# psipred/DMPfold2

Measured on AMD Instinct MI355X. Metric: structures/s at L=300, N_seq=2000, 10 iters+100 min, higher is better.
Workload: dtype f32 with full-width operands on the bf16 matrix cores (option precision = 2): convolution operands split exactly into 3 bf16 pieces (24 significand bits), the 6 piece products above 2^-24 accumulated in f32 by v_mfma_f32_32x32x16_bf16; vertical GRU the same way (3 bf16 pieces per operand, 6 products

## Files before the change

dmpfold2_amd/csrc/vgru_x3.hip:

```cpp
#include "vgru.h"

namespace dmp {

typedef __bf16 vx_bf16x8 __attribute__((ext_vector_type(8)));

__device__ __forceinline__ void vx_split8(const float (&w)[8], vx_bf16x8 (&p)[3]) {
  float r[8];
#pragma unroll
  for (int e = 0; e < 8; ++e) { const __bf16 h = (__bf16)w[e]; p[0][e] = h; r[e] = w[e] - (float)h; }
#pragma unroll
  for (int e = 0; e < 8; ++e) { const __bf16 h = (__bf16)r[e]; p[1][e] = h; r[e] = r[e] - (float)h; }
#pragma unroll
  for (int e = 0; e < 8; ++e) p[2][e] = (__bf16)r[e];
}

__device__ __forceinline__ vp_f32x4 vx_mfma(vx_bf16x8 a, vx_bf16x8 b, vp_f32x4 c) {
  return __builtin_amdgcn_mfma_f32_16x16x32_bf16(a, b, c, 0, 0, 0);
}

__device__ __forceinline__ float vx_sigmoid(float x) { return 1.0f / (1.0f + expf(-x)); }

constexpr int VX_KS = 4;
constexpr int VX_WQ = 6;
constexpr size_t VX_WQ_BYTES = (size_t)VP_GRID * 4 * VX_KS * VX_WQ * 64 * 16;
static_assert(4 * VX_KS * 3 * 2 * 64 == VP_WL0_SLOTS, "two pieces of layer 0's weights fill the LDS area of the f16 form's pieces");

constexpr int VX_SC1 = 16;

struct VxAddr {
  __amdgpu_buffer_rsrc_t r0, r1, rq;
  unsigned vlane, vq;
  unsigned k4w, krot, Lb;
};

__device__ __forceinline__ void vx_request(vp_f32x4 (&F)[4][2], int u4, unsigned S, unsigned col, const VxAddr& A) {
  const unsigned base = ((A.k4w + 8 * ((S + A.krot) & (VX_KS - 1))) * A.Lb + col + (u4 & 1) * 16) * 16;
#pragma unroll
  for (int h = 0; h < 2; ++h)
    F[u4][h] = __builtin_bit_cast(vp_f32x4, __builtin_amdgcn_raw_buffer_load_b128(u4 < 2 ? A.r1 : A.r0, A.vlane, base + h * A.Lb * 16, VX_SC1));
}

__device__ __forceinline__ void vx_split_octet(const vp_f32x4 (&f)[2], vx_bf16x8 (&q)[3]) {
  const float wv[8] = {f[0][0], f[0][1], f[0][2], f[0][3], f[1][0], f[1][1], f[1][2], f[1][3]};
  vx_split8(wv, q);
}

template <bool ACT0, bool ACT1>
__device__ __forceinline__ void vx_tile_products(vp_f32x4 (&a0)[3][2], vp_f32x4 (&a1)[4][2], const vx_bf16x8 (&PA)[VX_KS][3][3],
                                                 const vx_bf16x8 (&PB)[VX_KS][3][2], vx_bf16x8 (&WB)[3], vx_bf16x8 (&WC)[3],
                                                 const vx_bf16x8* __restrict__ wl0w, vp_f32x4 (&F)[4][2], vx_bf16x8 (&Q)[2][3],
                                                 const VxAddr& A, unsigned tcol, unsigned ncol) {
#pragma unroll
  for (int S = 0; S < VX_KS; ++S) {
    vx_bf16x8 T[3][2];
#pragma unroll
    for (int g = 0; g < 3; ++g) {
      T[g][0] = wl0w[((S * 3 + g) * 2 + 0) * 64];
      T[g][1] = wl0w[((S * 3 + g) * 2 + 1) * 64];
    }
    __builtin_amdgcn_sched_barrier(0);
#pragma unroll
    for (int u4 = 0; u4 < 4; ++u4) {
      const int unit = 4 * S + u4, nt = u4 & 1, cur = unit & 1, nxt = cur ^ 1, n4 = (u4 + 1) & 3;
      vx_bf16x8 (&P)[3] = Q[cur];
      const int nm = u4 < 2 ? (ACT1 ? 18 : 0) : (ACT0 ? 18 : 0) + (ACT1 ? 18 : 0);
#pragma unroll
      for (int pb = 2; pb >= 0; --pb)
#pragma unroll
        for (int pa = 2 - pb; pa >= 0; --pa)
#pragma unroll
          for (int g = 0; g < 3; ++g) {
            if (u4 < 2) {
              if (ACT1) a1[g][nt] = vx_mfma(pa == 2 ? WB[g] : PB[S][g][pa == 2 ? 0 : pa], P[pb], a1[g][nt]);
            } else {
              if (ACT0) a0[g][nt] = vx_mfma(pa == 2 ? WC[g] : T[g][pa == 2 ? 0 : pa], P[pb], a0[g][nt]);
              if (ACT1) a1[g == 2 ? 3 : g][nt] = vx_mfma(PA[S][g][pa], P[pb], a1[g == 2 ? 3 : g][nt]);
            }
          }
      vx_split_octet(F[n4], Q[nxt]);
      vx_request(F, n4, (unit + 5) >> 2 & (VX_KS - 1), unit + 5 < 4 * VX_KS ? tcol : ncol, A);
      if (u4 == 1) {
#pragma unroll
        for (int g = 0; g < 3; ++g)
          WB[g] = __builtin_bit_cast(vx_bf16x8, __builtin_amdgcn_raw_buffer_load_b128(A.rq, A.vq, (((S + 1) & (VX_KS - 1)) * VX_WQ + g) * 1024, 0));
      }
      if (u4 == 3) {
#pragma unroll
        for (int g = 0; g < 3; ++g)
          WC[g] = __builtin_bit_cast(vx_bf16x8, __builtin_amdgcn_raw_buffer_load_b128(A.rq, A.vq, (((S + 1) & (VX_KS - 1)) * VX_WQ + 3 + g) * 1024, 0));
      }
#pragma unroll
      for (int i = 0; i < 36; ++i)
        if (i < nm) {
          __builtin_amdgcn_sched_group_barrier(0x008, 1, 0);
          __builtin_amdgcn_sched_group_barrier(0x002, 3, 0);
        }
      __builtin_amdgcn_sched_barrier(0);
    }
  }
}

__global__ __launch_bounds__(256) __attribute__((amdgpu_waves_per_eu(1, 1)))
void vgru_persist_x3_kernel(VStaticF32 st, const VGroupRec* __restrict__ rec, VPSync* __restrict__ sync,
                            int* __restrict__ fault, int t_lo, int t_hi, int ntiles, int barrier) {
  extern __shared__ __attribute__((aligned(16))) unsigned char vx_smem[];
  vx_bf16x8* wl0 = reinterpret_cast<vx_bf16x8*>(vx_smem);
  vp_f32x4* red = reinterpret_cast<vp_f32x4*>(vx_smem + VP_WL0_SLOTS * 16);
  float* tab = reinterpret_cast<float*>(vx_smem + (VP_WL0_SLOTS + VP_RED_SLOTS) * 16);
  __shared__ int sh_u, sh_abort;
  __shared__ __attribute__((aligned(16))) float sh_bias[2][4][16];
  __shared__ int sh_tile[VP_MAX_XCD_TILES][5];
  __shared__ unsigned long long sh_msa[VG_MAX_MEMBERS];
  const int tid = threadIdx.x, lane = tid & 63;
  const int w = __builtin_amdgcn_readfirstlane(tid >> 6);
  unsigned xcc;
  if (barrier) {
    asm volatile("s_getreg_b32 %0, hwreg(HW_REG_XCC_ID)" : "=s"(xcc));
    xcc &= 7u;
    if (tid == 0) {
      sh_u = (int)__hip_atomic_fetch_add(&sync->count[xcc], 1u, __ATOMIC_RELAXED, __HIP_MEMORY_SCOPE_AGENT);
      sh_abort = 0;
    }
  } else {
    xcc = blockIdx.x & 7u;
    if (tid == 0) { sh_u = (int)(blockIdx.x >> 3); sh_abort = 0; }
  }
  __syncthreads();
  const int u = sh_u;
  if (u >= 32) {
    if (tid == 0) atomicOr(fault, DMP_FAULT_VGRU_HANDOFF);
    return;
  }
  const int j0 = 16 * u, lr = lane & 15, lq = lane >> 4;
  const int Lb = ntiles * VG_TB;
  const int c_lo = (int)(((long long)ntiles * xcc) / 8), c_hi = (int)(((long long)ntiles * (xcc + 1)) / 8);

  vx_bf16x8 PA[VX_KS][3][3], PB[VX_KS][3][2];
  uint4* wqw = st.wq + (size_t)(blockIdx.x * 4 + w) * VX_KS * VX_WQ * 64 + lane;
#pragma unroll
  for (int S = 0; S < VX_KS; ++S)
#pragma unroll
    for (int g = 0; g < 3; ++g) {
      float wa[8], wb[8], wc[8];
#pragma unroll
      for (int h = 0; h < 2; ++h) {
        const int64_t off = (int64_t)(g * 128 + 32 * w + 8 * ((S + u) & (VX_KS - 1)) + 2 * lq + h) * 512 + j0 + lr;
        const float4 a = st.wx1[off], b = st.wh1[off], c = st.wh0[off];
        wa[4 * h + 0] = a.x; wa[4 * h + 1] = a.y; wa[4 * h + 2] = a.z; wa[4 * h + 3] = a.w;
        wb[4 * h + 0] = b.x; wb[4 * h + 1] = b.y; wb[4 * h + 2] = b.z; wb[4 * h + 3] = b.w;
        wc[4 * h + 0] = c.x; wc[4 * h + 1] = c.y; wc[4 * h + 2] = c.z; wc[4 * h + 3] = c.w;
      }
      vx_split8(wa, PA[S][g]);
      vx_bf16x8 pb[3], pc[3];
      vx_split8(wb, pb);
      vx_split8(wc, pc);
      PB[S][g][0] = pb[0];
      PB[S][g][1] = pb[1];
      wl0[(((w * VX_KS + S) * 3 + g) * 2 + 0) * 64 + lane] = pc[0];
      wl0[(((w * VX_KS + S) * 3 + g) * 2 + 1) * 64 + lane] = pc[1];
      wqw[(S * VX_WQ + g) * 64] = __builtin_bit_cast(uint4, pb[2]);
      wqw[(S * VX_WQ + 3 + g) * 64] = __builtin_bit_cast(uint4, pc[2]);
    }
  asm volatile("s_waitcnt vmcnt(0)" ::: "memory");
  const vx_bf16x8* wl0w = wl0 + w * VX_KS * 3 * 2 * 64 + lane;
  if (tid < 128) sh_bias[tid >> 6][(tid >> 4) & 3][tid & 15] = st.bias[tid >> 6][((tid >> 4) & 3) * 512 + j0 + (tid & 15)];
  for (int i = tid; i < 3 * 22 * 16; i += 256) {
    const int g = i / (22 * 16), code = (i / 16) % 22, row = i & 15;
    tab[(g * 24 + code) * 16 + row] = st.wx0[(g * 22 + code) * 512 + j0 + row];
  }
  const int fl = __builtin_amdgcn_readfirstlane(tid >> 7), fg = (tid >> 5) & 3, fc = tid & 31;
  const int flane = 16 * fg + (fc & 15), fnt = fc >> 4;
  const int j4 = j0 + 4 * fg;
  const int nmem = rec->nmem;
  if (c_hi - c_lo > VP_MAX_XCD_TILES) {
    if (tid == 0) atomicOr(fault, DMP_FAULT_VGRU_HANDOFF);
    return;
  }
  for (int i = tid; i < c_hi - c_lo; i += 256) {
    const int tile = c_lo + (i + u) % (c_hi - c_lo);
    int mi = 0;
    for (int m = 1; m < VG_MAX_MEMBERS; ++m)
      if (m < nmem && tile >= rec->mem[m].tile0) mi = m;
    sh_tile[i][0] = rec->mem[mi].N;
    sh_tile[i][1] = rec->mem[mi].L;
    sh_tile[i][2] = (tile - rec->mem[mi].tile0) * VG_TB;
    sh_tile[i][3] = mi;
    sh_tile[i][4] = tile;
  }
  if (tid < VG_MAX_MEMBERS) sh_msa[tid] = tid < nmem ? (unsigned long long)rec->mem[tid].msa : 0ull;
  __syncthreads();
  auto next_active = [&](int ct, int t) {
    for (; ct < c_hi; ++ct) {
      const int N = __builtin_amdgcn_readfirstlane(sh_tile[ct - c_lo][0]);
      if (t < N || (t >= 1 && t <= N)) break;
    }
    return ct;
  };
  const unsigned state_bytes = (unsigned)(128 * Lb * 16);

  VxAddr A;
  A.k4w = (unsigned)(32 * w);
  A.krot = (unsigned)(u & (VX_KS - 1));
  A.Lb = (unsigned)Lb;
  A.vlane = (unsigned)((2 * lq * Lb + lr) * 16);
  A.vq = (unsigned)(lane * 16);
  A.rq = __builtin_amdgcn_make_buffer_rsrc(st.wq + (size_t)(blockIdx.x * 4 + w) * VX_KS * VX_WQ * 64, 0, VX_KS * VX_WQ * 1024, 0x00020000);
  vx_bf16x8 WB[3], WC[3];
#pragma unroll
  for (int g = 0; g < 3; ++g) {
    WB[g] = __builtin_bit_cast(vx_bf16x8, __builtin_amdgcn_raw_buffer_load_b128(A.rq, A.vq, g * 1024, 0));
    WC[g] = __builtin_bit_cast(vx_bf16x8, __builtin_amdgcn_raw_buffer_load_b128(A.rq, A.vq, (3 + g) * 1024, 0));
  }
  for (int t = t_lo; t < t_hi; ++t) {
    const int par = t & 1;
    A.r0 = __builtin_amdgcn_make_buffer_rsrc(st.hT[0][par], 0, state_bytes, 0x00020000);
    A.r1 = __builtin_amdgcn_make_buffer_rsrc(st.hT[1][par ^ 1], 0, state_bytes, 0x00020000);
    const __amdgpu_buffer_rsrc_t rh = fl ? A.r1 : A.r0;
    float* hnext = fl ? st.hT[1][par] : st.hT[0][par ^ 1];
    int ct = next_active(c_lo, t);
    vp_f32x4 F[4][2];
    vx_bf16x8 Q[2][3];
    if (ct < c_hi) {
      const unsigned col0 = (unsigned)(__builtin_amdgcn_readfirstlane(sh_tile[ct - c_lo][4]) * VG_TB);
#pragma unroll
      for (int u4 = 0; u4 < 4; ++u4) vx_request(F, u4, 0, col0, A);
      vx_split_octet(F[0], Q[0]);
      vx_request(F, 0, 1, col0, A);
    }
    while (ct < c_hi) {
      const int nx = next_active(ct + 1, t);
      const int ncol = __builtin_amdgcn_readfirstlane(sh_tile[(nx < c_hi ? nx : ct) - c_lo][4]) * VG_TB;
      const int N = __builtin_amdgcn_readfirstlane(sh_tile[ct - c_lo][0]);
      const int L = __builtin_amdgcn_readfirstlane(sh_tile[ct - c_lo][1]);
      const bool act0 = t < N, act1 = t >= 1 && t <= N;
      const int tcol = __builtin_amdgcn_readfirstlane(sh_tile[ct - c_lo][4]) * VG_TB;
      vp_f32x4 a0[3][2], a1[4][2];
#pragma unroll
      for (int g = 0; g < 3; ++g) { a0[g][0] = vp_f32x4{0, 0, 0, 0}; a0[g][1] = vp_f32x4{0, 0, 0, 0}; }
#pragma unroll
      for (int g = 0; g < 4; ++g) { a1[g][0] = vp_f32x4{0, 0, 0, 0}; a1[g][1] = vp_f32x4{0, 0, 0, 0}; }
      if (act0 && act1)
        vx_tile_products<true, true>(a0, a1, PA, PB, WB, WC, wl0w, F, Q, A, (unsigned)tcol, (unsigned)ncol);
      else if (act0)
        vx_tile_products<true, false>(a0, a1, PA, PB, WB, WC, wl0w, F, Q, A, (unsigned)tcol, (unsigned)ncol);
      else
        vx_tile_products<false, true>(a0, a1, PA, PB, WB, WC, wl0w, F, Q, A, (unsigned)tcol, (unsigned)ncol);
      const int b = tcol + fc;
      const int64_t hoff = ((int64_t)(j4 >> 2) * Lb + b) * 4;
      float hp[4];
#pragma unroll
      for (int i = 0; i < 4; ++i)
        hp[i] = __builtin_bit_cast(float, __builtin_amdgcn_raw_buffer_load_b32(rh, (unsigned)(hoff * 4 + 4 * i), 0, VX_SC1));
      const int bm = sh_tile[ct - c_lo][2] + fc;
      const uint8_t* msa = reinterpret_cast<const uint8_t*>(sh_msa[sh_tile[ct - c_lo][3]]);
      const int code = (fl == 0 && act0 && bm < L) ? (int)msa[(int64_t)t * L + bm] : 0;
#pragma unroll
      for (int g = 0; g < 3; ++g)
#pragma unroll
        for (int nt = 0; nt < 2; ++nt) red[(w * 14 + g * 2 + nt) * 64 + lane] = a0[g][nt];
#pragma unroll
      for (int g = 0; g < 4; ++g)
#pragma unroll
        for (int nt = 0; nt < 2; ++nt) red[(w * 14 + 6 + g * 2 + nt) * 64 + lane] = a1[g][nt];
      __syncthreads();
      if (fl ? act1 : act0) {
        const int nq = fl ? 4 : 3, base = fl ? 6 : 0;
        vp_f32x4 sum[4];
#pragma unroll
        for (int q = 0; q < 4; ++q) {
          if (q < nq) {
            const int a = base + q * 2 + fnt;
            sum[q] = ((red[(0 * 14 + a) * 64 + flane] + red[(1 * 14 + a) * 64 + flane]) + red[(2 * 14 + a) * 64 + flane]) +
                     red[(3 * 14 + a) * 64 + flane];
          }
        }
        if (fl == 0) {
          const float* tr = tab + (0 * 24 + code) * 16 + 4 * fg;
          const float* tz = tab + (1 * 24 + code) * 16 + 4 * fg;
          const float* tn = tab + (2 * 24 + code) * 16 + 4 * fg;
#pragma unroll
          for (int i = 0; i < 4; ++i) { sum[0][i] += tr[i]; sum[1][i] += tz[i]; sum[3][i] = tn[i]; }
        }
        const float* br = &sh_bias[fl][0][4 * fg];
        const float* bz = &sh_bias[fl][1][4 * fg];
        const float* bi = &sh_bias[fl][2][4 * fg];
        const float* bh = &sh_bias[fl][3][4 * fg];
        float hn[4];
#pragma unroll
        for (int i = 0; i < 4; ++i) {
          const float rg = vx_sigmoid(sum[0][i] + br[i]);
          const float zg = vx_sigmoid(sum[1][i] + bz[i]);
          const float ng = tanhf((sum[3][i] + bi[i]) + rg * (sum[2][i] + bh[i]));
          hn[i] = (hp[i] - ng) * zg + ng;
        }
        *reinterpret_cast<float4*>(hnext + hoff) = make_float4(hn[0], hn[1], hn[2], hn[3]);
      }
      __syncthreads();
      ct = nx;
    }
    if (!barrier) break;
    if (vp_row_barrier(sync, fault, xcc, u, w, lane, tid, t, t_lo, &sh_abort)) break;
  }
}

size_t vgru_x3_stream_bytes() { return VX_WQ_BYTES; }

int vgru_x3_kernel_attrs(dmp_ctx* c) {
  (void)c;
  DMP_HIP(hipFuncSetAttribute((const void*)vgru_persist_x3_kernel, hipFuncAttributeMaxDynamicSharedMemorySize, VP_LDS_BYTES));
  return DMP_OK;
}

int vgru_x3_group_steps(dmp_ctx* lead, int t_lo, int t_hi, hipStream_t s) {
  return vgru_f32_launch(vgru_persist_x3_kernel, lead, t_lo, t_hi, s);
}

}
```

Measured before the change: 4.383.

## Defer GRU gate epilogue of each tile to overlap with next tile's MFMA products

Instead of doing the cross-wave reduction and the GRU gate/state update right after each column tile, the epilogue is deferred and run after the next tile's matrix-core products. The goal is to hide reduction, sigmoid and tanh latency behind MFMA work and to drop one barrier stall per tile. In exchange it adds an extra __syncthreads per deferred tile, keeps more live state in registers, and forces the full both-active product path whenever an epilogue is pending.

```diff
diff --git a/dmpfold2_amd/csrc/vgru_x3.hip b/dmpfold2_amd/csrc/vgru_x3.hip
--- a/dmpfold2_amd/csrc/vgru_x3.hip
+++ b/dmpfold2_amd/csrc/vgru_x3.hip
@@ -43,6 +43,42 @@
 __device__ __forceinline__ void vx_split_octet(const vp_f32x4 (&f)[2], vx_bf16x8 (&q)[3]) {
   const float wv[8] = {f[0][0], f[0][1], f[0][2], f[0][3], f[1][0], f[1][1], f[1][2], f[1][3]};
   vx_split8(wv, q);
+}
+
+struct VxPend {
+  const vp_f32x4* rf;
+  const float* tabf;
+  const float* biasf;
+  bool l0;
+  float rg[4], zg[4], x[4];
+};
+
+__device__ __forceinline__ vp_f32x4 vx_pend_qsum(const VxPend& P, int q) {
+  return ((P.rf[(0 * 14 + 2 * q) * 64] + P.rf[(1 * 14 + 2 * q) * 64]) + P.rf[(2 * 14 + 2 * q) * 64]) + P.rf[(3 * 14 + 2 * q) * 64];
+}
+
+template <int STAGE>
+__device__ __forceinline__ void vx_pend_stage(VxPend& P) {
+  if (STAGE < 2) {
+    const vp_f32x4 s = vx_pend_qsum(P, STAGE);
+    const vp_f32x4 tg = *reinterpret_cast<const vp_f32x4*>(P.tabf + STAGE * 24 * 16);
+    const vp_f32x4 bg = *reinterpret_cast<const vp_f32x4*>(P.biasf + STAGE * 16);
+#pragma unroll
+    for (int i = 0; i < 4; ++i) {
+      const float v = P.l0 ? s[i] + tg[i] : s[i];
+      (STAGE == 0 ? P.rg : P.zg)[i] = vx_sigmoid(v + bg[i]);
+    }
+  } else {
+    const vp_f32x4 shn = vx_pend_qsum(P, 2), s3 = vx_pend_qsum(P, 3);
+    const vp_f32x4 tn = *reinterpret_cast<const vp_f32x4*>(P.tabf + 2 * 24 * 16);
+    const vp_f32x4 bi = *reinterpret_cast<const vp_f32x4*>(P.biasf + 2 * 16);
+    const vp_f32x4 bh = *reinterpret_cast<const vp_f32x4*>(P.biasf + 3 * 16);
+#pragma unroll
+    for (int i = 0; i < 4; ++i) {
+      const float s_in = P.l0 ? tn[i] : s3[i];
+      P.x[i] = (s_in + bi[i]) + P.rg[i] * (shn[i] + bh[i]);
+    }
+  }
 }
 
 template <bool ACT0, bool ACT1>
@@ -227,6 +263,10 @@
       vx_split_octet(F[0], Q[0]);
       vx_request(F, 0, 1, col0, A);
     }
+    int pend = -1, ptab = 0;
+    bool pact = false;
+    int64_t phoff = 0;
+    float php[4] = {0.0f, 0.0f, 0.0f, 0.0f};
     while (ct < c_hi) {
       const int nx = next_active(ct + 1, t);
       const int ncol = __builtin_amdgcn_readfirstlane(sh_tile[(nx < c_hi ? nx : ct) - c_lo][4]) * VG_TB;
@@ -239,12 +279,35 @@
       for (int g = 0; g < 3; ++g) { a0[g][0] = vp_f32x4{0, 0, 0, 0}; a0[g][1] = vp_f32x4{0, 0, 0, 0}; }
 #pragma unroll
       for (int g = 0; g < 4; ++g) { a1[g][0] = vp_f32x4{0, 0, 0, 0}; a1[g][1] = vp_f32x4{0, 0, 0, 0}; }
-      if (act0 && act1)
+      bool defer = false;
+      if (nx < c_hi) {
+        const int Nn = __builtin_amdgcn_readfirstlane(sh_tile[nx - c_lo][0]);
+        defer = t >= 1 && t < Nn;
+      }
+      VxPend P;
+      P.l0 = fl == 0;
+      P.rf = red + ((fl ? 6 : 0) + fnt) * 64 + flane;
+      P.tabf = tab + ptab;
+      P.biasf = &sh_bias[fl][0][4 * fg];
+      if (pend >= 0 || (act0 && act1))
         vx_tile_products<true, true>(a0, a1, PA, PB, WB, WC, wl0w, F, Q, A, (unsigned)tcol, (unsigned)ncol);
       else if (act0)
         vx_tile_products<true, false>(a0, a1, PA, PB, WB, WC, wl0w, F, Q, A, (unsigned)tcol, (unsigned)ncol);
       else
         vx_tile_products<false, true>(a0, a1, PA, PB, WB, WC, wl0w, F, Q, A, (unsigned)tcol, (unsigned)ncol);
+      if (pend >= 0) { vx_pend_stage<0>(P); vx_pend_stage<1>(P); vx_pend_stage<2>(P); }
+      if (pend >= 0) {
+        if (pact) {
+          float hn[4];
+#pragma unroll
+          for (int i = 0; i < 4; ++i) {
+            const float ng = tanhf(P.x[i]);
+            hn[i] = (php[i] - ng) * P.zg[i] + ng;
+          }
+          *reinterpret_cast<float4*>(hnext + phoff) = make_float4(hn[0], hn[1], hn[2], hn[3]);
+        }
+        __syncthreads();
+      }
       const int b = tcol + fc;
       const int64_t hoff = ((int64_t)(j4 >> 2) * Lb + b) * 4;
       float hp[4];
@@ -263,6 +326,17 @@
 #pragma unroll
         for (int nt = 0; nt < 2; ++nt) red[(w * 14 + 6 + g * 2 + nt) * 64 + lane] = a1[g][nt];
       __syncthreads();
+      if (defer) {
+        pend = ct - c_lo;
+        pact = fl ? act1 : act0;
+        phoff = hoff;
+        ptab = code * 16 + 4 * fg;
+#pragma unroll
+        for (int i = 0; i < 4; ++i) php[i] = hp[i];
+        ct = nx;
+        continue;
+      }
+      pend = -1;
       if (fl ? act1 : act0) {
         const int nq = fl ? 4 : 3, base = fl ? 6 : 0;
         vp_f32x4 sum[4];
```

Measured after the change: 4.407 (median of 6 runs). About the same (+0.5%).
